# hitbc/panSVR

Measured on AMD Instinct MI355X. Metric: signal reads realigned/sec (150 bp PE); bit-exact CIGAR vs CPU ref, higher is better.
Workload: dtype u8/int32 (2-bit k-mers, 8-bit DP deltas, 32-bit scores); 1 GPU; configs[1]: 1000000 synthetic 150 bp PE signal read pairs per GPU vs 10000-anchor SV reference (11.8 Mbp), `panSVR aln` hot path; pairs_per_gpu=1000000, engines_per_gpu=1, in_process_rebases=0, index_hbm_bytes=2713674320, index_distribution=every rank uploads its own copy from host memory

## Files before the change

### include/psvr_engine.h

```cpp
#ifndef PSVR_ENGINE_H_
#define PSVR_ENGINE_H_

#include <stddef.h>
#include <stdint.h>

#ifdef __cplusplus
extern "C" {
#endif

#define PSVR_OK                0
#define PSVR_ERR_ARG           1
#define PSVR_ERR_UNSUPPORTED   2
#define PSVR_ERR_DEVICE        3
#define PSVR_ERR_NOMEM         4
#define PSVR_ERR_IO            5
#define PSVR_ERR_OVERFLOW      6

const char *psvr_last_error(void);
int psvr_device_count(void);
void *psvr_host_alloc(size_t bytes);
void psvr_host_free(void *p);
int psvr_device_warmup(int device, int n_streams);

#define PSVR_KSW_NEG_INF (-0x40000000)
#define PSVR_EZ_SCORE_ONLY  0x01
#define PSVR_EZ_RIGHT       0x02
#define PSVR_EZ_GENERIC_SC  0x04
#define PSVR_EZ_APPROX_MAX  0x08
#define PSVR_EZ_APPROX_DROP 0x10
#define PSVR_EZ_EXTZ_ONLY   0x40
#define PSVR_EZ_REV_CIGAR   0x80

typedef struct psvr_extz {
	int32_t max, zdropped;
	int32_t max_q, max_t;
	int32_t mqe, mqe_t;
	int32_t mte, mte_q;
	int32_t score;
	int32_t n_cigar;
	int32_t reach_end;
	int32_t reserved;
	int64_t cigar_off;
} psvr_extz_t;

typedef struct psvr_ksw_params {
	int8_t  m;
	int8_t  mat[25];
	int8_t  q, e, q2, e2;
	int32_t w;
	int32_t zdrop;
	int32_t end_bonus;
	int32_t flag;
} psvr_ksw_params_t;

static inline int64_t psvr_cigar_bound(int32_t qlen, int32_t tlen) { return (int64_t)qlen + tlen + 2; }

int psvr_extd2_batch(int device, int64_t n,
                     const uint8_t *qseq, const int64_t *q_off, const int32_t *qlen,
                     const uint8_t *tseq, const int64_t *t_off, const int32_t *tlen,
                     const psvr_ksw_params_t *par,
                     psvr_extz_t *ez, uint32_t *cigar_arena, int64_t cigar_cap);

int psvr_extz2_batch(int device, int64_t n,
                     const uint8_t *qseq, const int64_t *q_off, const int32_t *qlen,
                     const uint8_t *tseq, const int64_t *t_off, const int32_t *tlen,
                     const psvr_ksw_params_t *par,
                     psvr_extz_t *ez, uint32_t *cigar_arena, int64_t cigar_cap);

typedef struct psvr_dp_plan psvr_dp_plan_t;
int psvr_dp_plan_create(int device, int64_t n, const int32_t *qlen_host, const int32_t *tlen_host,
                        const psvr_ksw_params_t *par, int variant , psvr_dp_plan_t **plan);
int64_t psvr_dp_plan_workspace_bytes(const psvr_dp_plan_t *plan);
int psvr_dp_plan_launch(psvr_dp_plan_t *plan,
                        const uint8_t *d_qseq, const int64_t *d_q_off,
                        const uint8_t *d_tseq, const int64_t *d_t_off,
                        psvr_extz_t *d_ez, uint32_t *d_cigar_arena, void *d_work, void *stream);
int psvr_dp_plan_describe(const psvr_dp_plan_t *plan, char *buf, size_t buflen);
void psvr_dp_plan_destroy(psvr_dp_plan_t *plan);

typedef struct psvr_dp_regime {
	int32_t skip;
	int32_t swapped;
	int32_t nowrap_ok;
	int32_t zdrop_inert;
	int32_t long_thres;
	int32_t qe_shift;
} psvr_dp_regime_t;
int psvr_dp_regime(const psvr_ksw_params_t *par, int variant , psvr_dp_regime_t *out);


typedef struct psvr_index psvr_index_t;

typedef struct psvr_index_view {
	const uint64_t *ref_seq;  uint64_t n_ref_seq;
	const uint64_t *seq;      uint64_t n_seq;
	const uint64_t *seqf;     uint64_t n_seqf;
	const uint64_t *pos;      uint64_t n_pos;
	const uint64_t *posp;     uint64_t n_posp;
	const uint64_t *hash;     uint64_t n_hash;
	const uint32_t *kmer;     uint64_t n_kmer;
	const uint64_t *off;      uint64_t n_off;
	const char *chr_text;
	const char *const *header_names; int32_t n_header;
} psvr_index_view_t;

int psvr_index_create(const psvr_index_view_t *view, int device, psvr_index_t **out);
int psvr_index_create_from_device(const psvr_index_view_t *view, int device, psvr_index_t **out);
int psvr_index_load(const char *index_dir, const char *header_sam, int device, psvr_index_t **out);
int psvr_index_clone(const psvr_index_t *src, int device, psvr_index_t **out);
int psvr_index_build(const char *anchors_fa, const char *header_sam, int device, psvr_index_t **out);
void psvr_index_destroy(psvr_index_t *idx);
int64_t psvr_index_device_bytes(const psvr_index_t *idx);
int32_t psvr_index_n_anchor(const psvr_index_t *idx);
const char *psvr_index_sv_print_string(const psvr_index_t *idx, int32_t sv_id);
const char *psvr_index_sv_vcf_id(const psvr_index_t *idx, int32_t sv_id);

int psvr_seed_search_kmer_batch(const psvr_index_t *idx, int64_t n, const uint64_t *kmers, int64_t *range, uint8_t *found);
typedef struct psvr_vertex_mem {
	uint64_t uid;
	uint32_t seed_id;
	uint32_t read_pos, uni_pos_off, length, pos_n;
	uint32_t right_i;
} psvr_vertex_mem_t;
int psvr_seed_mem_batch(const psvr_index_t *idx, int64_t n, const uint64_t *kmer_index, const uint64_t *read_bits, int64_t n_words,
                        const int64_t *word_off, const uint32_t *read_off, const uint32_t *read_len, psvr_vertex_mem_t *out);

typedef struct psvr_engine psvr_engine_t;

typedef struct psvr_aln_params {
	int32_t match, mismatch, gap_open, gap_ex, gap_open2, gap_ex2, zdrop;
	int32_t normal_read_length, isize_min, isize_max;
	int32_t min_filter_score;
} psvr_aln_params_t;
void psvr_aln_params_default(psvr_aln_params_t *p);

typedef struct psvr_ori {
	int32_t  chr_id;
	uint32_t ref_bg, read_bg, align_score;
	uint8_t  mapq, direction , unmapped, reserved;
} psvr_ori_t;

#define PSVR_MAX_RESULT 12
typedef struct psvr_cand {
	uint32_t align_score, chain_score, ref_bg, read_bg;
	int32_t  chr_id, sv_id;
	uint32_t max_index;
	uint32_t n_cigar;
	int64_t  cigar_off;
	uint8_t  direction, mapq, reserved[6];
} psvr_cand_t;

typedef struct psvr_read_result {
	int32_t n_result;
	uint8_t unmapped, early_out, is_str, reserved;
	int32_t primary, secondary;
	int32_t has_mate, mate_chr_id;
	uint32_t mate_ref_bg;
	int32_t prim_sv_id, mate_sv_id;
	uint32_t n_seed[2];
	uint32_t reserved1;
	uint64_t seed_hash[2], chain_hash[2];
	psvr_cand_t cand[PSVR_MAX_RESULT];
} psvr_read_result_t;

typedef struct psvr_read_hdr {
	int32_t n_result;
	uint8_t unmapped, early_out, is_str, reserved;
	int32_t primary, secondary;
	int32_t has_mate, mate_chr_id;
	uint32_t mate_ref_bg;
	int32_t prim_sv_id, mate_sv_id;
	int32_t reserved2;
	int64_t cand_off;
} psvr_read_hdr_t;

typedef struct psvr_pair_result {
	int32_t max_score, cur_isize;
	int32_t proper, gain;
	int32_t max1, max2;
} psvr_pair_result_t;

int psvr_engine_create(const psvr_index_t *idx, const psvr_aln_params_t *par, psvr_engine_t **out);
void psvr_engine_destroy(psvr_engine_t *eng);
int psvr_engine_align_batch(psvr_engine_t *eng, int64_t n_pairs, const char *bases, const int64_t *base_off,
                            const psvr_ori_t *ori, psvr_read_result_t *reads, psvr_pair_result_t *pairs,
                            uint32_t *cigar, int64_t cigar_cap, int trace);
int psvr_engine_upload(psvr_engine_t *eng, int64_t n_pairs, const char *bases, const int64_t *base_off, const psvr_ori_t *ori);
int psvr_engine_run(psvr_engine_t *eng, int trace, void *stream);
int psvr_engine_download(psvr_engine_t *eng, psvr_read_result_t *reads, psvr_pair_result_t *pairs,
                         uint32_t *cigar, int64_t cigar_cap, int64_t *cigar_used);
int psvr_engine_download_compact(psvr_engine_t *eng, psvr_read_hdr_t *hdr, psvr_pair_result_t *pairs,
                                 psvr_cand_t *cands, int64_t cand_cap, int64_t *cand_used,
                                 uint32_t *cigar, int64_t cigar_cap, int64_t *cigar_used);
int psvr_engine_set_stream_pos(psvr_engine_t *eng, const int64_t pos[3]);
int psvr_engine_stream_end(psvr_engine_t *eng, int64_t end[3]);
int psvr_engine_rebase(psvr_engine_t *eng, const int64_t pos[3], void *stream);
int psvr_engine_stats(const psvr_engine_t *eng, char *buf, size_t buflen);

typedef struct psvr_fastq psvr_fastq_t;
typedef struct psvr_fastq_info {
	int64_t n_pairs, used_bytes, total_bases, n_lines;
	int32_t stop;
	int32_t reserved;
} psvr_fastq_info_t;
int  psvr_fastq_create(int device, psvr_fastq_t **out);
int  psvr_fastq_parse(psvr_fastq_t *fq, const char *text, int64_t n_bytes, int at_end,
                      int64_t max_pairs, int64_t max_bases, psvr_fastq_info_t *info);
int  psvr_fastq_download(const psvr_fastq_t *fq, uint64_t *line_start, uint16_t *name_end,
                         int64_t *base_off, psvr_ori_t *ori, char *bases);
int  psvr_engine_upload_fastq(psvr_engine_t *eng, const psvr_fastq_t *fq, int64_t first_pair, int64_t n_pairs);
void psvr_fastq_destroy(psvr_fastq_t *fq);

typedef struct psvr_bam_emit psvr_bam_emit_t;
typedef struct psvr_bam_emit_info { int64_t n_bytes, n_records, n_written_pairs, n_declined_pairs; } psvr_bam_emit_info_t;
#define PSVR_EMIT_NOT_ORI 1
int  psvr_bam_emit_create(const psvr_index_t *idx, psvr_bam_emit_t **out);
int  psvr_bam_emit_results(psvr_bam_emit_t *em, const psvr_fastq_t *fq, int64_t first_pair, int64_t n_pairs,
                           const psvr_read_hdr_t *hdr, const psvr_pair_result_t *pairs, const psvr_cand_t *cands, int64_t n_cands,
                           const uint32_t *cigar, int64_t n_cigar, int32_t flags, psvr_bam_emit_info_t *info);
int  psvr_bam_emit_engine(psvr_bam_emit_t *em, psvr_engine_t *eng, const psvr_fastq_t *fq, int32_t flags, psvr_bam_emit_info_t *info);
int  psvr_bam_emit_download(const psvr_bam_emit_t *em, void *bytes, int64_t cap, int64_t *pair_off, uint8_t *pair_state);
void psvr_bam_emit_destroy(psvr_bam_emit_t *em);

int64_t psvr_bgzf_bound(int64_t n_bytes);
int psvr_bgzf_compress(int device, const void *in, int64_t n_bytes, void *out, int64_t out_cap, int64_t *out_bytes);

int64_t psvr_bgzf_members_bound(int64_t n_bytes, int32_t member_bytes);
int psvr_bgzf_compress_members(int device, const void *in, int64_t n_bytes, int32_t member_bytes,
                               void *out, int64_t out_cap, int64_t *out_bytes,
                               int64_t *member_off, int64_t member_cap, int64_t *n_members);

int psvr_bgzf_decompress(int device, const void *in, int64_t n_bytes, int64_t *in_used,
                         void *out, int64_t out_cap, int64_t *out_bytes,
                         int64_t *member_off, int64_t member_cap, int64_t *n_members, int64_t *bad_member);

int psvr_sort_order_u64(int device, int64_t n, const uint64_t *keys, uint32_t *order);

#ifdef __cplusplus
}
#endif
#endif
```

### pansvr_amd/csrc/aln_device.h

```cpp
#pragma once
#include <stdint.h>
#include "../../include/psvr_engine.h"

#if defined(__HIPCC__)
#include <hip/hip_runtime.h>
#define PSVR_HD __host__ __device__ __forceinline__
#define PSVR_HDN __host__ __device__
#else
#define PSVR_HD inline
#define PSVR_HDN
#endif

namespace psvr {

static const int kLenKmer = 20, kSeedStep = 5, kUniPosNMax = 32;
static const int kMaxOut = 6;
static const int kMaxReadLen = 1600;
static const int kFwd = 1, kRev = 0;
static const int kSegMax = 160;
static const int kCigMax = 256;
static const int kMemSlot = 32;

struct SvDev { uint32_t chr_id; uint32_t st_pos; int32_t end_offset; int32_t pad; };

// ... 14 lines not shown
};

PSVR_HD void hash_pair(const DevIndex &ix, uint64_t h, uint64_t &lo, uint64_t &hi);

struct VMem { uint64_t uid; uint32_t seed_id, read_pos, uni_pos_off, length, pos_n, pad; };
struct VU { uint64_t uid; uint32_t read_pos, uni_pos_off, length1, length2, pos_n, cov; };
struct USeed { uint32_t read_begin, read_end, seed_id, ref_begin, ref_end, cov; };
struct PathN { int32_t dist, pre_node; uint32_t brk; uint32_t used; };

static const int kArenaTopStride = 32, kArenaMaxShards = 16;
template <class T> struct Arena {
	T *base;
	unsigned long long *top;
	unsigned long long cap;
	int *overflow;
	unsigned int nshard;
};

PSVR_HD unsigned long long atomic_bump(unsigned long long *p, unsigned long long n)
{
#if defined(__HIP_DEVICE_COMPILE__)
	return atomicAdd(p, n);
#else
	unsigned long long o = *p;
	*p += n;
	return o;
#endif
}

template <class T> PSVR_HD long long arena_alloc(const Arena<T> &a, unsigned long long n)
{
#if defined(__HIP_DEVICE_COMPILE__)
	if (a.nshard > 1) {
		const unsigned long long cap_s = a.cap / a.nshard;
		for (unsigned int k = 0; k < a.nshard; ++k) {
			const unsigned long long s = (blockIdx.x + k) % a.nshard;
			if (k && a.top[s * kArenaTopStride] + n > cap_s) continue;
			const unsigned long long o = atomic_bump(a.top + s * kArenaTopStride, n);
			if (o + n <= cap_s) return (long long)(s * cap_s + o);
		}
		*a.overflow = 1;
		return -1;
	}
#endif
	unsigned long long o = atomic_bump(a.top, n);
	if (o + n > a.cap) { *a.overflow = 1; return -1; }
	return (long long)o;
}

struct Strand {
	long long mem_off; uint32_t mem_n;
	long long us_off;  uint32_t us_n;
	uint64_t seed_hash, chain_hash;
};

struct ChainCand {
	uint32_t chain_score, max_index, read_bg, ref_bg;
	int32_t chr_id;
	int32_t direction;
};

struct Seg {
	int32_t kind;
	int32_t a, b;
};

struct DpDesc {
	int32_t read, strand;
	int32_t q_st, qlen;
	uint32_t ref_st; int32_t tlen;
	int32_t type;
	int32_t pad;
};

struct CandWork {
	int32_t read, k;
	int32_t n_seg;
	int32_t read_score;
	int32_t rba;
	int32_t bad;
	long long seg_off;
};

struct Ctx {
	DevIndex idx;
	psvr_aln_params_t par;
	int8_t mat[25];
	long long n_pairs;
	const char *bases; const long long *base_off; const psvr_ori_t *ori;
	int32_t lmax;
	int32_t wmax;
	const int32_t *grand; long long grand_n; long long grand_base;
	const int32_t *hrand[2]; long long hrand_n; long long hrand_base[2];
	long long n_slots;
	const int32_t *src;
	long long *poff;
	int32_t *rcnt;
	long long *hoff; int32_t *hcnt;
	const uint8_t *force;
	uint8_t *active; uint8_t *unmapped; uint8_t *is_str; uint8_t *has_n4;
	uint8_t *has_mem;
	int32_t *str_list; unsigned int *str_cnt;
	int32_t *read_l;
	uint8_t *bin;
	uint64_t *rb;
	uint8_t *seed_list;
	Strand *strand;
	ChainCand *ccand; int32_t *n_ccand;
	psvr_read_hdr_t *rh; psvr_pair_result_t *pres;
	psvr_cand_t *cand;
	Arena<VMem> mem; Arena<USeed> us; PathN *path;
	Arena<Seg> seg; Arena<DpDesc> dp; Arena<CandWork> cw; Arena<uint32_t> cig;
	const psvr_extz_t *dp_ez; const uint32_t *dp_cig;
	const uint8_t *tseq_in; int32_t *stale_open;
	int32_t *any_h;
	int32_t trace;
	int32_t *err;
	unsigned long long *stats;
};

enum { ST_PROBES = 0, ST_HITS, ST_SEEDS, ST_DP, ST_SIMPLE, ST_CELLS, ST_READS, ST_CAND, ST_N };

PSVR_HD void stat_add(const Ctx &c, int k, unsigned long long v)
{
	if (!c.stats) return;
#if defined(__HIP_DEVICE_COMPILE__)
	atomicAdd(c.stats + k, v);
#else
	c.stats[k] += v;
#endif
}

PSVR_HD long long src_read(const Ctx &c, long long read)
{
	return c.src ? (long long)c.src[read >> 1] * 2 + (read & 1) : read;
}

PSVR_HD uint64_t fnv1a(uint64_t h, uint64_t v)
{
	for (int i = 0; i < 8; ++i) { h ^= (v >> (8 * i)) & 0xff; h *= 1099511628211ULL; }
	return h;
}

PSVR_HD bool bucket_occupied(const DevIndex &ix, uint64_t h)
{
#ifdef PSVR_EMU_SPARSE_HASH
	(void)ix, (void)h;
	return true;
#else
	return !ix.occ || ((ix.occ[h >> 5] >> (h & 31)) & 1u);
#endif
}

PSVR_HD void bloom_slot(uint64_t kmer, uint32_t shift, uint64_t &word, uint64_t &mask)
{
	const uint64_t h = kmer * 0x9E3779B97F4A7C15ull;
	const uint64_t g = (h ^ (h >> 32)) * 0xD6E8FEB86659FD93ull;
	word = h >> shift;
	mask = (1ull << (g >> 58)) | (1ull << ((g >> 52) & 63)) | (1ull << ((g >> 46) & 63));
}
PSVR_HD bool kmer_maybe_present(const DevIndex &ix, uint64_t kmer)
{
#ifdef PSVR_EMU_SPARSE_HASH
	(void)ix, (void)kmer;
	return true;
#else
	if (ix.bloom) {
		uint64_t w, m;
		bloom_slot(kmer, ix.bloom_shift, w, m);
		return (ix.bloom[w] & m) == m;
	}
	return bucket_occupied(ix, kmer >> 12);
#endif
}

PSVR_HD void hash_pair(const DevIndex &ix, uint64_t h, uint64_t &lo, uint64_t &hi)
{
#ifdef PSVR_EMU_SPARSE_HASH
	auto at = [&](uint64_t x) {
		uint64_t l = 0, r = ix.sp_n;
		while (l < r) { uint64_t m = (l + r) >> 1; if (ix.sp_id[m] < x) l = m + 1; else r = m; }
		return l < ix.sp_n ? ix.sp_start[l] : ix.n_kmer;
	};
	lo = at(h), hi = at(h + 1);
#else
	lo = ix.hash[h], hi = ix.hash[h + 1];
#endif
}

PSVR_HD int base_at(const uint64_t *w, uint64_t i) { return (int)((w[i >> 5] >> ((31 - (i & 0x1f)) << 1)) & 3); }

PSVR_HD uint64_t window32(const uint64_t *w, uint64_t i)
{
	uint64_t k = i >> 5, sh = (i & 31) << 1;
	uint64_t a = w[k];
	return sh ? (a << sh) | (w[k + 1] >> (64 - sh)) : a;
}
PSVR_HD int mismatches_packed(const uint64_t *A, uint64_t ia, const uint64_t *B, uint64_t ib, int len, int cap)
{
	int nm = 0;
	for (int j = 0; j < len && nm < cap; j += 128) {
		const uint64_t ka = (ia + (uint64_t)j) >> 5, kb = (ib + (uint64_t)j) >> 5;
		const unsigned sa = (unsigned)((ia + (uint64_t)j) & 31) << 1, sb = (unsigned)((ib + (uint64_t)j) & 31) << 1;
		const int rem = len - j, nw = rem >= 128 ? 4 : (rem + 31) >> 5;
		uint64_t wa[5], wb[5];
#if defined(__HIP_DEVICE_COMPILE__)
#pragma unroll
#endif
		for (int q = 0; q < 5; ++q) { const bool in = q <= nw; wa[q] = in ? A[ka + q] : 0, wb[q] = in ? B[kb + q] : 0; }
#if defined(__HIP_DEVICE_COMPILE__)
#pragma unroll
#endif
		for (int q = 0; q < 4; ++q) {
			if (q >= nw) break;
			const uint64_t xa = sa ? (wa[q] << sa) | (wa[q + 1] >> (64 - sa)) : wa[q], xb = sb ? (wb[q] << sb) | (wb[q + 1] >> (64 - sb)) : wb[q];
			uint64_t x = xa ^ xb;
			x = (x | (x >> 1)) & 0x5555555555555555ull;
			const int r = rem - 32 * q;
			if (r < 32) x &= ~0ull << ((32 - r) << 1);
#if defined(__HIP_DEVICE_COMPILE__)
			nm += __popcll(x);
#else
			nm += __builtin_popcountll(x);
#endif
		}
	}
	return nm < cap ? nm : cap;
}

PSVR_HDN inline void prep_read(const Ctx &c, long long read)
{
	const long long sr = src_read(c, read);
	const psvr_ori_t &o = c.ori[sr];
	const int L = (int)(c.base_off[sr + 1] - c.base_off[sr]);
	c.read_l[read] = L;
	bool unm = o.unmapped != 0;
	if ((uint32_t)o.chr_id > 24u) unm = true;
	c.unmapped[read] = unm;
	c.is_str[read] = 0, c.has_mem[read] = 0;
	long long item = (read >> 1) * 3 + (read & 1);
	c.rcnt[item] = 0;
	c.hcnt[read] = 0;
	c.n_ccand[read] = 0;
	for (int s = 0; s < 2; ++s) { Strand &st = c.strand[read * 2 + s]; st.mem_n = st.us_n = 0; st.mem_off = st.us_off = 0; st.seed_hash = st.chain_hash = 1469598103934665603ULL; }
	if (L > kMaxReadLen || L < kLenKmer) { c.active[read] = 0; if (L > kMaxReadLen) *c.err = 1; return; }
	if (!unm && o.align_score == (uint32_t)(L * c.par.match)) { c.active[read] = 0; return; }
	c.active[read] = 1;
	const char *s = c.bases + c.base_off[sr];
	uint8_t *b0 = c.bin + (read * 2) * (long long)c.lmax, *b1 = b0 + c.lmax;
	uint64_t *w0 = c.rb + (read * 2) * (long long)c.wmax, *w1 = w0 + c.wmax;
	for (int i = 0; i < c.wmax; ++i) w0[i] = 0, w1[i] = 0;
	long long ro = c.poff[read >> 1] + ((read & 1) ? c.rcnt[(read >> 1) * 3] : 0);
	int draws = 0;
	for (int i = 0; i < L; ++i) {
		char ch = s[i];
		if (ch == 'N') {
			long long k = ro + draws - c.grand_base;
			int32_t r;
			if (c.force && draws < (int)c.force[4 * read]) r = c.force[4 * read + 1 + draws];
			else r = (k >= 0 && k < c.grand_n) ? c.grand[k] : (*c.err = 2, 0);
			ch = "ACGT"[r % 4];
			++draws;
		}
		uint8_t code = (ch == 'C' || ch == 'c') ? 1 : (ch == 'G' || ch == 'g') ? 2 : (ch == 'T' || ch == 't') ? 3 : (ch == 'n') ? 4 : 0;
		b0[i] = code;
		b1[L - 1 - i] = code ^ 3;
	}
	for (int i = 0; i < L; ++i) {
		w0[i >> 5] |= ((uint64_t)b0[i]) << ((31 - (i & 0x1f)) << 1);
		w1[i >> 5] |= ((uint64_t)b1[i]) << ((31 - (i & 0x1f)) << 1);
	}
	c.rcnt[item] = draws;
	{ uint8_t any4 = 0; for (int i = 0; i < L; ++i) any4 |= b0[i] > 3; c.has_n4[read] = any4; }
	stat_add(c, ST_READS, 1);
}

PSVR_HD uint64_t get_kmer(uint32_t off, const uint64_t *rb)
{
	uint32_t w = off >> 5, iw = off & 0x1f;
	uint64_t full = (rb[w] << (iw << 1)) | (iw == 0 ? 0 : (rb[w + 1] >> ((32 - iw) << 1)));
	return full >> ((32 - kLenKmer) << 1);
}

PSVR_HDN inline void str_detect(const Ctx &c, long long read)
{
	if (!c.active[read]) return;
	const int L = c.read_l[read];
	const uint64_t *rb = c.rb + (read * 2) * (long long)c.wmax;
	uint8_t *sl = c.seed_list + read * (long long)c.lmax;
	const uint32_t kn = L - kLenKmer + 1;
	uint32_t distinct = 0;
	for (uint32_t i = 0; i < kn; ++i) {
		uint64_t ki = get_kmer(i, rb);
		bool first = true;
		for (uint32_t j = 0; j < i; ++j) if (get_kmer(j, rb) == ki) { first = false; break; }
		distinct += first;
	}
	if (!(distinct < kn - 15)) { c.is_str[read] = 0; return; }
	c.is_str[read] = 1;
	for (uint32_t i = 0; i < kn; ++i) {
		uint64_t ki = get_kmer(i, rb);
		int cnt = 0;
		for (uint32_t j = 0; j < kn; ++j) cnt += get_kmer(j, rb) == ki;
		sl[i] = cnt >= 4 ? 0 : 1;
	}
	int bg = 0, ed = 0;
	for (uint32_t o = 0; o < (uint32_t)kSeedStep; ++o) {
		bg += sl[o] == 0, ed += sl[L - kLenKmer - o] == 0;
		sl[o] += 2, sl[L - kLenKmer - o] += 4;
	}
	if (bg < kSeedStep && ed < kSeedStep) {
		int tot = 0;
		for (uint32_t o = 0; tot < kSeedStep && o < kn; ++o) {
			if (sl[o] > 0) continue;
			sl[o] += 8, tot++;
		}
	}
}

PSVR_HD uint8_t seed_list_at(const uint8_t *sl, int len, int rev, int i)
{
	if (!rev) return sl[i];
	if (!(len & 1) && (i == len / 2 || i == len / 2 - 1)) return sl[i];
	return sl[len - 1 - i];
}

PSVR_HD int clz64(uint64_t x)
{
#if defined(__HIP_DEVICE_COMPILE__)
	return __clzll((long long)x);
#else
	return __builtin_clzll(x);
#endif
}
PSVR_HD int ctz64(uint64_t x)
{
#if defined(__HIP_DEVICE_COMPILE__)
	return __ffsll((unsigned long long)x) - 1;
#else
	return __builtin_ctzll(x);
#endif
}
PSVR_HD uint32_t match_right(const uint64_t *A, uint64_t ia, const uint64_t *B, uint64_t ib, uint32_t max)
{
	uint32_t n = 0;
	while (n < max) {
		const uint64_t ka = (ia + n) >> 5;
		const unsigned sa = (unsigned)((ia + n) & 31) << 1;
		const uint32_t rem = max - n;
		const int nw = rem >= 128 ? 4 : (int)((rem + 31) >> 5);
		uint64_t wa[5];
#if defined(__HIP_DEVICE_COMPILE__)
#pragma unroll
#endif
		for (int q = 0; q < 5; ++q) wa[q] = (q < nw || (q == nw && sa != 0)) ? A[ka + q] : 0;
#if defined(__HIP_DEVICE_COMPILE__)
#pragma unroll
#endif
		for (int q = 0; q < 4; ++q) {
			if (q >= nw) break;
			const uint64_t xa = sa ? (wa[q] << sa) | (wa[q + 1] >> (64 - sa)) : wa[q];
			uint64_t x = xa ^ window32(B, ib + n + 32u * (uint32_t)q);
			x = (x | (x >> 1)) & 0x5555555555555555ull;
			const uint32_t left = rem - 32u * (uint32_t)q, lim = left < 32 ? left : 32;
			if (x) { const uint32_t k = (uint32_t)clz64(x) >> 1; return n + 32u * (uint32_t)q + (k < lim ? k : lim); }
		}
		n += rem < 128 ? rem : 128;
	}
	return max;
}
PSVR_HD uint32_t match_left(const uint64_t *A, uint64_t ia, const uint64_t *B, uint64_t ib, uint32_t max)
{
	uint32_t n = 0;
	while (n < max) {
		uint32_t lim = max - n < 32 ? max - n : 32;
		uint64_t x = window32(A, ia - n - lim) ^ window32(B, ib - n - lim);
		x = (x | (x >> 1)) & 0x5555555555555555ull;
		if (lim < 32) x &= ~0ull << ((32 - lim) << 1);
		if (x) { uint32_t k = ((uint32_t)ctz64(x) - ((32 - lim) << 1)) >> 1; return n + k; }
		n += lim;
	}
	return max;
}

PSVR_HD uint32_t probe_kmer(const DevIndex &ix, uint64_t kmer, uint64_t &first_hit)
{
	const uint64_t key = kmer & 0xfff, h = kmer >> 12;
	uint64_t lo, hi;
	hash_pair(ix, h, lo, hi);
	long long l = 0, r = (long long)(hi - lo) - 1, first = -1, last = -1;
	const uint32_t *v = ix.kmer + lo;
	while (l <= r) {
		long long m = (l + r) / 2;
		uint32_t t = v[m] >> 4;
		if (t == key) {
			first = last = m;
			long long sl2 = l, sr = m - 1;
			while (sl2 <= sr) { long long sm = (sl2 + sr) / 2; uint32_t t2 = v[sm] >> 4; if (t2 == key) first = sm, sr = sm - 1; else if (t2 > key) sr = sm - 1; else sl2 = sm + 1; }
			sl2 = m + 1, sr = r;
			while (sl2 <= sr) { long long sm = (sl2 + sr) / 2; uint32_t t2 = v[sm] >> 4; if (t2 == key) last = sm, sl2 = sm + 1; else if (t2 > key) sr = sm - 1; else sl2 = sm + 1; }
			break;
		} else if (t > key) r = m - 1;
		else l = m + 1;
	}
	if (first < 0) return 0;
	first_hit = lo + (uint64_t)first;
	return (uint32_t)(last - first + 1);
}

PSVR_HDN inline HitRec hit_record(const DevIndex &ix, uint64_t hit)
{
	HitRec h;
	const uint64_t kp = ix.off[hit];
	long long lo2 = 0, hi2 = (long long)ix.n_seqf - 1, uid = -1;
	if (ix.uid_hint) {
		const uint64_t b = kp >> ix.uid_shift;
		lo2 = (long long)ix.uid_hint[b], hi2 = (long long)ix.uid_hint[b + 1];
	}
	while (lo2 <= hi2) {
		long long mid = (lo2 + hi2) >> 1;
		uint64_t sv = ix.seqf[mid];
		if (kp < sv) hi2 = mid - 1;
		else if (kp > sv) lo2 = mid + 1;
		else { uid = mid; break; }
	}
	if (uid < 0) uid = hi2;
	const uint64_t f0 = ix.seqf[uid], f1 = ix.seqf[uid + 1];
	h.kp = kp, h.uid = (uint32_t)uid, h.ul = (uint32_t)(kp - f0), h.ur = (uint32_t)(f1 - (kp + kLenKmer));
	h.pos_n = (uint32_t)(ix.posp[uid + 1] - ix.posp[uid]), h.pad[0] = h.pad[1] = 0;
	return h;
}
PSVR_HD uint32_t mem_for_hit(const DevIndex &ix, uint64_t hit, const uint64_t *rb, uint32_t off, int L, VMem &m)
{
	const HitRec h = ix.hitrec ? ix.hitrec[hit] : hit_record(ix, hit);
	const uint64_t kp = h.kp, uid = h.uid;
	const uint32_t ul = h.ul, ur = h.ur;
	const uint32_t lmax = ul < off ? ul : off, rmax0 = (uint32_t)(L - (int)off - kLenKmer), rmax = ur < rmax0 ? ur : rmax0;
	const uint32_t li = 1 + match_left(ix.seq, kp, rb, off, lmax);
	const uint32_t ri = 1 + match_right(ix.seq, kp + kLenKmer, rb, (uint64_t)off + kLenKmer, rmax);
	m.uid = (uint64_t)uid, m.seed_id = 0, m.read_pos = off + 1 - li, m.uni_pos_off = ul + 1 - li;
	m.length = kLenKmer + li + ri - 2, m.pos_n = h.pos_n, m.pad = 0;
	return ri;
}

template <bool LOCAL> PSVR_HD void seed_strand_t(const Ctx &c, long long rs, const uint64_t *rb_local)
{
	const long long read = rs >> 1;
	const int rev = (int)(rs & 1);
	if (!c.active[read]) return;
	const int L = c.read_l[read];
	const uint64_t *rb = LOCAL ? rb_local : c.rb + rs * (long long)c.wmax;
	const uint8_t *sl = c.seed_list + read * (long long)c.lmax;
	const bool is_str = c.is_str[read] != 0;
	const uint32_t kn = L - kLenKmer + 1;
	const DevIndex &ix = c.idx;
	long long base = rs * (long long)kMemSlot;
	uint32_t total = 0, probes = 0;
	for (int pass = 0; pass < 3; ++pass) {
		if (pass == 1) continue;
		uint32_t n = 0, msr = 0, off = 0, nh = 0;
		uint64_t kmer = 0, first_hit = 0;
		int stage = 0;
		for (;;) {
			while (stage != 2 && off < kn) {
				while (off < kn) {
					if (off + kLenKmer - 1 <= msr || (is_str && seed_list_at(sl, (int)kn, rev, off) == 0)) { off += kSeedStep; continue; }
					if (pass == 0) ++probes;
					kmer = get_kmer(off, rb);
					if (kmer_maybe_present(ix, kmer)) { stage = 1; break; }
					off += kSeedStep;
				}
				if (stage != 1) break;
				nh = probe_kmer(ix, kmer, first_hit);
				if (nh == 0 || nh > (uint32_t)kUniPosNMax) { off += kSeedStep; stage = 0; }
				else stage = 2;
			}
			if (stage != 2) break;
			uint32_t mri = 1;
			for (uint64_t hit = first_hit; hit < first_hit + nh; ++hit) {
				VMem m;
				const uint32_t ri = mem_for_hit(ix, hit, rb, off, L, m);
				m.seed_id = n;
				if (pass == 2 || n < (uint32_t)kMemSlot) c.mem.base[base + n] = m;
				++n;
				if (ri > mri) mri = ri;
			}
			msr = off + kLenKmer + mri - 1;
			off += kSeedStep;
			stage = 0;
		}
		if (pass == 0) {
			total = n;
			if (n <= (uint32_t)kMemSlot) break;
			base = arena_alloc(c.mem, n);
			if (base < 0) return;
		}
	}
	Strand &st = c.strand[rs];
	st.mem_off = base, st.mem_n = total;
	if (total) c.has_mem[read] = 1;
	if (c.stats) { stat_add(c, ST_PROBES, probes); stat_add(c, ST_HITS, total); }
}
PSVR_HDN inline void seed_strand(const Ctx &c, long long rs) { seed_strand_t<false>(c, rs, nullptr); }

template <class T, class Less> PSVR_HD void stable_sort(T *a, T *tmp, uint32_t n, Less less)
{
	if (n < 2) return;
	if (n <= 16) {
		for (uint32_t i = 1; i < n; ++i) {
			T x = a[i];
			uint32_t j = i;
			while (j > 0 && less(x, a[j - 1])) { a[j] = a[j - 1]; --j; }
			a[j] = x;
		}
		return;
	}
	T *src = a, *dst = tmp;
	for (uint32_t w = 1; w < n; w <<= 1) {
		for (uint32_t lo = 0; lo < n; lo += 2 * w) {
			uint32_t mid = lo + w < n ? lo + w : n, hi = lo + 2 * w < n ? lo + 2 * w : n;
			uint32_t i = lo, j = mid, k = lo;
			while (i < mid && j < hi) { if (less(src[j], src[i])) dst[k++] = src[j++]; else dst[k++] = src[i++]; }
			while (i < mid) dst[k++] = src[i++];
			while (j < hi) dst[k++] = src[j++];
		}
		T *t = src; src = dst; dst = t;
	}
	if (src != a) for (uint32_t i = 0; i < n; ++i) a[i] = src[i];
}

PSVR_HDN inline void chain_strand(const Ctx &c, long long rs, int &hdraw_total)
{
	const long long read = rs >> 1;
	const int rev = (int)(rs & 1);
	if (!c.active[read]) return;
	Strand &st = c.strand[rs];
	const uint32_t mem_i = st.mem_n;
	VMem *vm = c.mem.base + st.mem_off;
	const DevIndex &ix = c.idx;
	if (mem_i > 1) {
		VMem *mtmp = nullptr;
		if (mem_i > 16) {
			long long t = arena_alloc(c.mem, mem_i);
			if (t < 0) return;
			mtmp = c.mem.base + t;
		}
		stable_sort(vm, mtmp, mem_i, [](const VMem &a, const VMem &b) { return a.uid != b.uid ? a.uid < b.uid : a.read_pos < b.read_pos; });
	}
	long long ubase = 0;
	uint32_t total = 0;
	const long long hro = c.hoff[read] + hdraw_total;
	int hdraw = 0;
	for (int pass = 0; pass < 2; ++pass) {
		uint32_t n = 0, vu_i = 0;
		hdraw = 0;
		bool stop = false;
		uint32_t j = 0;
		while (j < mem_i && !stop) {
			VU u;
			if (mem_i == 1) {
				const VMem &m = vm[0];
				u.uid = m.uid, u.read_pos = m.read_pos, u.uni_pos_off = m.uni_pos_off, u.length1 = u.length2 = m.length, u.pos_n = m.pos_n, u.cov = m.length;
				j = 1;
			} else {
				uint32_t s1 = j, cov = vm[s1].length;
				const uint64_t uid_t = vm[s1].uid;
				j++;
				while (j < mem_i && uid_t == vm[j].uid && vm[j].uni_pos_off > vm[j - 1].uni_pos_off) {
					int diff = (int)(vm[j].read_pos - vm[j - 1].read_pos - vm[j - 1].length);
					if (diff > 3) break;
					int ce = (int)((vm[j].uni_pos_off - vm[j - 1].uni_pos_off) - (vm[j].read_pos - vm[j - 1].read_pos));
					if ((ce < 0 ? -ce : ce) < 1) { cov += (diff > 0) ? vm[j].length : (uint32_t)(diff + (int)vm[j].length); ++j; }
					else break;
				}
				uint32_t e1 = j - 1;
				u.uid = vm[s1].uid, u.read_pos = vm[s1].read_pos, u.uni_pos_off = vm[s1].uni_pos_off, u.pos_n = vm[s1].pos_n, u.cov = cov;
				if (s1 == e1) u.length1 = u.length2 = vm[s1].length;
				else {
					u.length1 = vm[e1].read_pos + vm[e1].length - vm[s1].read_pos;
					u.length2 = vm[e1].uni_pos_off + vm[e1].length - vm[s1].uni_pos_off;
				}
			}
			uint32_t cnt = u.pos_n;
			bool sample = false;
			if (u.pos_n > 500) {
				if (u.pos_n > 8000) { stop = true; break; }
				cnt = 500, sample = true;
			}
			for (uint32_t k = 0; k < cnt; ++k) {
				uint32_t m = k;
				if (sample) {
					long long q = hro + hdraw - c.hrand_base[read & 1];
					int32_t rv = (q >= 0 && q < c.hrand_n) ? c.hrand[read & 1][q] : (*c.err = 3, 0);
					m = (uint32_t)rv % u.pos_n;
					++hdraw;
				}
				if (pass == 1) {
					USeed &s = c.us.base[ubase + n];
					s.seed_id = vu_i, s.read_begin = u.read_pos, s.read_end = u.read_pos + u.length1 - 1;
					s.ref_begin = (uint32_t)(ix.pos[m + ix.posp[u.uid]] + u.uni_pos_off - 1);
					s.ref_end = s.ref_begin + u.length2 - 1, s.cov = u.cov;
				}
				++n;
			}
			++vu_i;
		}
		if (pass == 0) {
			total = n;
			if (n == 0) break;
			ubase = arena_alloc(c.us, 2ull * n);
			if (ubase < 0) return;
		}
	}
	(void)rev;
	st.us_off = ubase, st.us_n = total;
	hdraw_total += hdraw;
	if (total == 0) return;
	USeed *v = c.us.base + ubase;
	PathN *pa = c.path + ubase;
	stable_sort(v, v + total, total, [](const USeed &a, const USeed &b) { return a.ref_end != b.ref_end ? a.ref_end < b.ref_end : a.ref_begin < b.ref_begin; });
	const bool is_str = c.is_str[read] != 0;
	const int max_ref_dis = is_str ? 400 : 50, max_read_dis = is_str ? 400 : 50;
// ... 1147 lines not shown
```

### pansvr_amd/csrc/engine.hip

```cpp
#include <hip/hip_runtime.h>
#include <algorithm>
#include <cstring>
#include <mutex>
#include <string>
#include <thread>
#include <vector>
#include "common.h"
#include "engine_core.h"
#include "bam_emit_hooks.h"
#include "fastq_parsed.h"
#include "host_io.h"
#include "index_build.h"
#include "ksw_device.h"
#include "ksw_launch.h"
#include "scan.h"

namespace psvr {

int dp_params(const psvr_ksw_params_t *par, int variant, DpParams *P);

static const int kBlock = 256;
static inline unsigned grid_for(long long n, int block = kBlock) { return (unsigned)((n + block - 1) / block); }

__device__ __forceinline__ long long pair_of(const int32_t *work, long long i) { return work ? (long long)work[i] : i; }
// ... 1744 lines not shown
	bi.ref_seq.resize(bi.ref_seq.size());
	psvr_index_view_t v;
	memset(&v, 0, sizeof v);
	v.ref_seq = bi.ref_seq.data(), v.n_ref_seq = bi.ref_seq.size(), v.seq = bi.seqb.data(), v.n_seq = bi.seqb.size();
	v.seqf = bi.seqf.data(), v.n_seqf = bi.seqf.size(), v.pos = bi.pos.data(), v.n_pos = bi.pos.size(), v.posp = bi.posp.data(), v.n_posp = bi.posp.size();
	v.hash = nullptr, v.n_hash = ((uint64_t)1 << 28) + 1, v.kmer = bi.kmer.data(), v.n_kmer = bi.kmer.size(), v.off = bi.off.data(), v.n_off = bi.off.size();
	std::vector<uint32_t> sid(bi.hash_sparse_id.size()), scn(bi.hash_sparse_cnt.size());
	for (size_t i = 0; i < sid.size(); ++i) sid[i] = (uint32_t)bi.hash_sparse_id[i], scn[i] = (uint32_t)bi.hash_sparse_cnt[i];
	int rc = index_upload(ix, &v, sid.data(), scn.data(), (long long)sid.size());
	if (rc) { delete ix; return rc; }
	*out = ix;
	return PSVR_OK;
}

extern "C" int psvr_index_load(const char *dir, const char *header_sam, int device, psvr_index_t **out)
{
	if (!dir || !header_sam || !out) return set_error(PSVR_ERR_ARG, "psvr_index_load: null argument");
	if (psvr_device_count() <= 0) return set_error(PSVR_ERR_DEVICE, "no HIP device visible: the engine has no CPU path");
	psvr_index *ix = new psvr_index;
	ix->device = device;
	std::string err;
	ix->host.defer_dense = true;
	if (!ix->host.load_dir(dir, header_sam, &err)) { delete ix; return set_error(PSVR_ERR_IO, "%s", err.c_str()); }
	HostIndex &h = ix->host;
	psvr_index_view_t v;
	memset(&v, 0, sizeof v);
	v.ref_seq = h.ref_seq.data(), v.n_ref_seq = h.ref_seq.size(), v.seq = h.seq.data(), v.n_seq = h.seq.size();
	v.seqf = h.seqf.data(), v.n_seqf = h.seqf.size(), v.pos = h.pos.data(), v.n_pos = h.pos.size(), v.posp = h.posp.data(), v.n_posp = h.posp.size();
	v.hash = h.hash.data(), v.n_hash = h.hash.size(), v.kmer = h.kmer.data(), v.n_kmer = h.kmer.size(), v.off = h.off.data(), v.n_off = h.off.size();
	int rc;
	if (!h.sparse_pairs.empty()) {
		const size_t ns = h.sparse_pairs.size() / 2;
		std::vector<uint32_t> sid(ns), scn(ns);
		for (size_t i = 0; i < ns; ++i) sid[i] = h.sparse_pairs[2 * i], scn[i] = h.sparse_pairs[2 * i + 1];
		{
			unsigned long long tot = 0;
			bool ok = true;
			for (size_t i = 0; i < ns && ok; ++i) { ok = sid[i] < (1u << 28) && (i == 0 || sid[i] > sid[i - 1]); tot += scn[i]; }
			if (!ok || tot != (unsigned long long)h.kmer.size()) { delete ix; return set_error(PSVR_ERR_IO, "unipath_g.hash.sparse: bucket ids must be < 4^14 and ascending, counts must add up to the %zu entries of unipath_g.kmer", h.kmer.size()); }
		}
		v.hash = nullptr, v.n_hash = ((uint64_t)1 << 28) + 1;
		rc = index_upload(ix, &v, sid.data(), scn.data(), (long long)ns);
		std::vector<uint32_t>().swap(h.sparse_pairs);
	} else rc = index_upload(ix, &v);
	std::vector<uint64_t>().swap(h.hash);
	if (rc) { delete ix; return rc; }
	*out = ix;
	return PSVR_OK;
}

extern "C" int psvr_index_clone(const psvr_index_t *src, int device, psvr_index_t **out)
{
	if (!src || !out) return set_error(PSVR_ERR_ARG, "psvr_index_clone: null argument");
	psvr_index *ix = new psvr_index;
	ix->device = device;
	ix->host = src->host;
	hipError_t he = hipSetDevice(device);
	auto cp = [&](DevBuf &d, const DevBuf &s0) {
		if (he != hipSuccess || !s0.p) return;
		he = d.alloc(s0.bytes);
		if (he == hipSuccess) he = hipMemcpyPeer(d.p, device, s0.p, src->device, s0.bytes);
		ix->bytes += (int64_t)s0.bytes;
	};
	cp(ix->ref_seq, src->ref_seq), cp(ix->seq, src->seq), cp(ix->seqf, src->seqf), cp(ix->pos, src->pos), cp(ix->posp, src->posp), cp(ix->hash, src->hash);
	cp(ix->off, src->off), cp(ix->kmer, src->kmer), cp(ix->chr_end, src->chr_end), cp(ix->chr_idx, src->chr_idx), cp(ix->sv, src->sv), cp(ix->occ, src->occ), cp(ix->uid_hint, src->uid_hint), cp(ix->bloom, src->bloom), cp(ix->hitrec, src->hitrec);
	if (he == hipSuccess) he = hipDeviceSynchronize();
	if (he != hipSuccess) { delete ix; return set_error(PSVR_ERR_DEVICE, "psvr_index_clone: %s", hipGetErrorString(he)); }
	DevIndex &d = ix->dev;
	d = src->dev;
	d.ref_seq = ix->ref_seq.as<uint64_t>(), d.seq = ix->seq.as<uint64_t>(), d.seqf = ix->seqf.as<uint64_t>(), d.pos = ix->pos.as<uint64_t>();
	d.posp = ix->posp.as<uint64_t>(), d.hash = ix->hash.as<uint64_t>(), d.off = ix->off.as<uint64_t>(), d.kmer = ix->kmer.as<uint32_t>();
	d.chr_end_n = ix->chr_end.as<uint32_t>(), d.chr_search_index = ix->chr_idx.as<uint32_t>(), d.sv = ix->sv.as<SvDev>();
	d.occ = ix->occ.as<uint32_t>(), d.uid_hint = ix->uid_hint.as<uint32_t>();
	if (src->bloom.p) d.bloom = ix->bloom.as<uint64_t>();
	if (src->hitrec.p) d.hitrec = ix->hitrec.as<HitRec>();
	*out = ix;
	return PSVR_OK;
}

extern "C" void psvr_index_destroy(psvr_index_t *ix) { delete ix; }
extern "C" int64_t psvr_index_device_bytes(const psvr_index_t *ix) { return ix ? ix->bytes : 0; }
extern "C" int32_t psvr_index_n_anchor(const psvr_index_t *ix) { return ix ? ix->host.chr_file_n : 0; }
extern "C" const char *psvr_index_sv_print_string(const psvr_index_t *ix, int32_t sv)
{
	return ix && sv >= 0 && sv < (int)ix->host.svh.size() ? ix->host.svh[sv].vcf_print_string.c_str() : nullptr;
}
extern "C" const char *psvr_index_sv_vcf_id(const psvr_index_t *ix, int32_t sv)
{
	return ix && sv >= 0 && sv < (int)ix->host.svh.size() ? ix->host.svh[sv].vcf_id.c_str() : nullptr;
}

__global__ __launch_bounds__(kBlock) void k_b3_search_kmer(DevIndex ix, long long n, const uint64_t *kmers, long long *range, uint8_t *found)
{
	const long long i = blockIdx.x * (long long)blockDim.x + threadIdx.x;
	if (i >= n) return;
	const uint64_t kmer = kmers[i] & 0xffffffffffull;
	uint64_t first = 0;
	const uint32_t nh = kmer_maybe_present(ix, kmer) ? probe_kmer(ix, kmer, first) : 0;
	found[i] = nh != 0;
	range[2 * i] = nh ? (long long)first : 0, range[2 * i + 1] = nh ? (long long)(first + nh - 1) : -1;
}
__global__ __launch_bounds__(kBlock) void k_b3_mem(DevIndex ix, long long n, const uint64_t *kmer_index, const uint64_t *read_bits, const long long *word_off, const uint32_t *read_off,
                                                   const uint32_t *read_len, psvr_vertex_mem_t *out)
{
	const long long i = blockIdx.x * (long long)blockDim.x + threadIdx.x;
	if (i >= n) return;
	VMem m;
	const uint32_t ri = mem_for_hit(ix, kmer_index[i], read_bits + word_off[i], read_off[i], (int)read_len[i], m);
	psvr_vertex_mem_t &o = out[i];
	o.uid = m.uid, o.seed_id = 0, o.read_pos = m.read_pos, o.uni_pos_off = m.uni_pos_off, o.length = m.length, o.pos_n = m.pos_n, o.right_i = ri;
}

extern "C" int psvr_seed_search_kmer_batch(const psvr_index_t *ix, int64_t n, const uint64_t *kmers, int64_t *range, uint8_t *found)
{
	if (!ix || n < 0 || (n && (!kmers || !range || !found))) return set_error(PSVR_ERR_ARG, "psvr_seed_search_kmer_batch: bad argument");
	if (n == 0) return PSVR_OK;
	PSVR_HIP(hipSetDevice(ix->device));
	DevBuf dk, dr, df;
	PSVR_HIP(dk.alloc((size_t)n * 8)); PSVR_HIP(dr.alloc((size_t)n * 16)); PSVR_HIP(df.alloc((size_t)n));
	PSVR_HIP(hipMemcpy(dk.p, kmers, (size_t)n * 8, hipMemcpyHostToDevice));
	hipLaunchKernelGGL(k_b3_search_kmer, dim3(grid_for(n)), dim3(kBlock), 0, nullptr, ix->dev, (long long)n, dk.as<uint64_t>(), dr.as<long long>(), df.as<uint8_t>());
	PSVR_HIP(hipGetLastError());
	PSVR_HIP(hipMemcpy(range, dr.p, (size_t)n * 16, hipMemcpyDeviceToHost));
	PSVR_HIP(hipMemcpy(found, df.p, (size_t)n, hipMemcpyDeviceToHost));
	return PSVR_OK;
}

extern "C" int psvr_seed_mem_batch(const psvr_index_t *ix, int64_t n, const uint64_t *kmer_index, const uint64_t *read_bits, int64_t n_words, const int64_t *word_off,
                                   const uint32_t *read_off, const uint32_t *read_len, psvr_vertex_mem_t *out)
{
	if (!ix || n < 0 || n_words < 0 || (n && (!kmer_index || !read_bits || !word_off || !read_off || !read_len || !out))) return set_error(PSVR_ERR_ARG, "psvr_seed_mem_batch: bad argument");
	if (n == 0) return PSVR_OK;
	const uint64_t n_index = ix->off.bytes / 8;
	for (int64_t i = 0; i < n; ++i) {
		const int64_t words = ((int64_t)read_len[i] + 31) / 32 + 1;
		if (kmer_index[i] >= n_index || word_off[i] < 0 || word_off[i] + words > n_words || read_len[i] < (uint32_t)kLenKmer || read_off[i] + (uint32_t)kLenKmer > read_len[i])
			return set_error(PSVR_ERR_ARG, "psvr_seed_mem_batch: item %lld is out of range (index entry, word window or read offset)", (long long)i);
	}
	PSVR_HIP(hipSetDevice(ix->device));
	DevBuf dk, db, dw, dro, drl, dout;
	PSVR_HIP(dk.alloc((size_t)n * 8)); PSVR_HIP(db.alloc((size_t)(n_words + 2) * 8)); PSVR_HIP(dw.alloc((size_t)n * 8)); PSVR_HIP(dro.alloc((size_t)n * 4)); PSVR_HIP(drl.alloc((size_t)n * 4));
	PSVR_HIP(dout.alloc((size_t)n * sizeof(psvr_vertex_mem_t)));
	PSVR_HIP(hipMemset((char *)db.p + (size_t)n_words * 8, 0, 16));
	PSVR_HIP(hipMemcpy(dk.p, kmer_index, (size_t)n * 8, hipMemcpyHostToDevice)); PSVR_HIP(hipMemcpy(db.p, read_bits, (size_t)n_words * 8, hipMemcpyHostToDevice));
	PSVR_HIP(hipMemcpy(dw.p, word_off, (size_t)n * 8, hipMemcpyHostToDevice)); PSVR_HIP(hipMemcpy(dro.p, read_off, (size_t)n * 4, hipMemcpyHostToDevice));
	PSVR_HIP(hipMemcpy(drl.p, read_len, (size_t)n * 4, hipMemcpyHostToDevice));
	hipLaunchKernelGGL(k_b3_mem, dim3(grid_for(n)), dim3(kBlock), 0, nullptr, ix->dev, (long long)n, dk.as<uint64_t>(), db.as<uint64_t>(), dw.as<long long>(), dro.as<uint32_t>(), drl.as<uint32_t>(),
	                   dout.as<psvr_vertex_mem_t>());
	PSVR_HIP(hipGetLastError());
	PSVR_HIP(hipMemcpy(out, dout.p, (size_t)n * sizeof(psvr_vertex_mem_t), hipMemcpyDeviceToHost));
	return PSVR_OK;
}

extern "C" int psvr_device_warmup(int device, int n_streams)
{
	if (device < 0 || device >= 64 || n_streams < 1) return set_error(PSVR_ERR_ARG, "psvr_device_warmup: bad argument");
	if (n_streams > 16) n_streams = 16;
	std::thread([device, n_streams]() {
		if (hipSetDevice(device) != hipSuccess) return;
		std::vector<hipStream_t> got;
		void *h = nullptr, *d = nullptr;
		const bool buf = hipHostMalloc(&h, 4096, hipHostMallocDefault) == hipSuccess && hipMalloc(&d, 4096) == hipSuccess;
		if (buf) memset(h, 0, 4096);
		for (int i = 0; i < n_streams; ++i) {
			hipStream_t s = nullptr;
			if (hipStreamCreateWithFlags(&s, hipStreamNonBlocking) != hipSuccess) break;
			if (buf) (void)hipMemcpyAsync(d, h, 4096, hipMemcpyHostToDevice, s), (void)hipMemsetAsync(d, 0, 4096, s), (void)hipMemcpyAsync(h, d, 4096, hipMemcpyDeviceToHost, s);
			(void)hipStreamSynchronize(s);
			got.push_back(s);
		}
		if (h) (void)hipHostFree(h);
		if (d) (void)hipFree(d);
		(void)hipGetLastError();
		StreamPool &P = stream_pool();
		std::lock_guard<std::mutex> lk(P.mu);
		for (hipStream_t s : got) P.idle[device].push_back(s);
	}).detach();
	return PSVR_OK;
}

struct psvr_engine {
	const psvr_index *ix;
	GpuBE be;
	EngineCore<GpuBE, GpuBE> core;
	bool committed = true;
	DevBuf full_out, cmp_cnt_c, cmp_cnt_w, cmp_off_c, cmp_off_w, cmp_hdr, cmp_cand, cmp_cig;
	bool compact_valid = false;
	long long compact_nc = 0, compact_nw = 0;
	hipStream_t own = nullptr;
	const psvr_fastq *src_fq = nullptr;
	int64_t src_first = 0, src_n = 0;
	uint64_t src_generation = 0;
	bool ran = false;
	explicit psvr_engine(const psvr_index *i) : ix(i), core(be) {}
};

extern "C" void psvr_aln_params_default(psvr_aln_params_t *p) { if (p) aln_params_default(p); }

extern "C" int psvr_engine_create(const psvr_index_t *ix, const psvr_aln_params_t *par, psvr_engine_t **out)
{
	if (!ix || !par || !out) return set_error(PSVR_ERR_ARG, "psvr_engine_create: null argument");
	PSVR_HIP(hipSetDevice(ix->device));
	psvr_engine *e = new psvr_engine(ix);
	e->own = stream_pool().get(ix->device);
	e->be.stream = e->own, e->be.device = ix->device;
	e->core.init(ix->dev, *par);
	*out = e;
	return PSVR_OK;
}

extern "C" void psvr_engine_destroy(psvr_engine_t *e)
{
	if (!e) return;
	(void)hipSetDevice(e->ix->device);
	const int dev = e->ix->device;
	hipStream_t own = e->own;
	delete e;
	stream_pool().put(dev, own);
}

static int engine_status(psvr_engine *e, int rc)
{
	if (e->be.last != hipSuccess) { hipError_t x = e->be.last; e->be.last = hipSuccess; return set_error(PSVR_ERR_DEVICE, "HIP error: %s", hipGetErrorString(x)); }
	if (rc) return set_error(rc, "%s", e->core.err.empty() ? psvr_last_error() : e->core.err.c_str());
	return PSVR_OK;
}

extern "C" int psvr_engine_upload(psvr_engine_t *e, int64_t n_pairs, const char *bases, const int64_t *base_off, const psvr_ori_t *ori)
{
	if (!e || n_pairs < 0 || (n_pairs && (!bases || !base_off || !ori))) return set_error(PSVR_ERR_ARG, "psvr_engine_upload: bad argument");
	PSVR_HIP(hipSetDevice(e->ix->device));
	e->be.stream = e->own;
	if (!e->committed) { e->core.commit(); e->committed = true; }
	e->compact_valid = false;
	e->src_fq = nullptr, e->ran = false;
	int rc = e->core.upload(n_pairs, bases, base_off, ori);
	return engine_status(e, rc);
}

extern "C" int psvr_engine_upload_fastq(psvr_engine_t *e, const psvr_fastq_t *fq, int64_t first_pair, int64_t n_pairs)
{
	if (psvr_device_count() <= 0) return set_error(PSVR_ERR_DEVICE, "no HIP device visible: the engine has no CPU path");
	if (!e || !fq || !fq->valid || first_pair < 0 || n_pairs < 0 || first_pair + n_pairs > fq->last.n_pairs) return set_error(PSVR_ERR_ARG, "psvr_engine_upload_fastq: bad argument");
	if (fq->device != e->ix->device)
		return set_error(PSVR_ERR_ARG, "psvr_engine_upload_fastq: the text was parsed on device %d, the engine runs on device %d (the bases would have to travel between them)", fq->device, e->ix->device);
	PSVR_HIP(hipSetDevice(e->ix->device));
	e->be.stream = e->own;
	if (!e->committed) { e->core.commit(); e->committed = true; }
	e->compact_valid = false;
	e->src_fq = nullptr, e->ran = false;
	const int64_t *off = fq->base_off.as<int64_t>() + 2 * first_pair;
	long long b0 = 0, b1 = fq->last.total_bases;
	const bool whole = first_pair == 0 && n_pairs == fq->last.n_pairs;
	if (!whole && n_pairs > 0 && !e->be.d2h({{&b0, off, 8}, {&b1, off + 2 * n_pairs, 8}})) return engine_status(e, PSVR_ERR_DEVICE);
	const int rc = e->core.upload_device(n_pairs, fq->bases.as<char>(), off, fq->ori.as<psvr_ori_t>() + 2 * first_pair, b0, b1 - b0);
	const int st = engine_status(e, rc);
	if (!st) e->src_fq = fq, e->src_first = first_pair, e->src_n = n_pairs, e->src_generation = fq->generation;
	return st;
}

extern "C" int psvr_engine_run(psvr_engine_t *e, int trace, void *stream)
{
	if (!e) return set_error(PSVR_ERR_ARG, "psvr_engine_run: null engine");
	PSVR_HIP(hipSetDevice(e->ix->device));
	e->be.stream = stream ? (hipStream_t)stream : e->own;
	e->be.timing = (trace & 4) != 0;
	e->be.timed.clear();
	e->compact_valid = false;
	int rc = e->core.run(trace & 1, (trace & 2) != 0);
	hipError_t s = hipStreamSynchronize(e->be.stream);
	if (s != hipSuccess) e->be.note(s);
	e->be.synced();
	e->be.collect_timing();
	e->committed = false;
	const int st = engine_status(e, rc);
	e->ran = st == PSVR_OK;
	return st;
}

extern "C" int psvr_engine_set_stream_pos(psvr_engine_t *e, const int64_t pos[3])
{
	if (!e || !pos) return set_error(PSVR_ERR_ARG, "psvr_engine_set_stream_pos: null argument");
	PSVR_HIP(hipSetDevice(e->ix->device));
	e->core.have_run = false, e->committed = true;
	e->core.grand_pos = pos[0], e->core.hrand_pos[0] = pos[1], e->core.hrand_pos[1] = pos[2];
	return PSVR_OK;
}

extern "C" int psvr_engine_stream_end(psvr_engine_t *e, int64_t end[3])
{
	if (!e || !end) return set_error(PSVR_ERR_ARG, "psvr_engine_stream_end: null argument");
	PSVR_HIP(hipSetDevice(e->ix->device));
	long long t[3];
	e->core.stream_end(t);
	end[0] = t[0], end[1] = t[1], end[2] = t[2];
	return engine_status(e, PSVR_OK);
}

extern "C" int psvr_engine_rebase(psvr_engine_t *e, const int64_t pos[3], void *stream)
{
	if (!e || !pos) return set_error(PSVR_ERR_ARG, "psvr_engine_rebase: null argument");
	PSVR_HIP(hipSetDevice(e->ix->device));
	e->be.stream = stream ? (hipStream_t)stream : e->own;
	e->compact_valid = false;
	int rc = e->core.rebase(pos[0], pos[1], pos[2], e->core.c.trace, false);
	hipError_t s = hipStreamSynchronize(e->be.stream);
// ... 132 lines not shown
```

Baseline: 356.5 million reads/s.

## Probe canonical bloom once per k-mer pair and share answers across strand lanes

The bloom filter is now keyed on the canonical (min of forward and reverse-complement) 20-mer, with separate bit masks for the two orientations, so one word fetch answers presence for a k-mer and its reverse complement. Forward and reverse strand threads of a read split the seed offsets between them, batch five bloom loads at a time to overlap memory latency, and exchange the other strand's answers through a lane shuffle. The seeding loop then reads a precomputed answer bitmask instead of probing the filter per offset. This adds reverse-complement arithmetic and assumes the paired strand lanes are adjacent and both active. It also adds a host API to read back the filter.

```diff
diff --git a/include/psvr_engine.h b/include/psvr_engine.h
--- a/include/psvr_engine.h
+++ b/include/psvr_engine.h
@@ -124,6 +124,7 @@
 } psvr_vertex_mem_t;
 int psvr_seed_mem_batch(const psvr_index_t *idx, int64_t n, const uint64_t *kmer_index, const uint64_t *read_bits, int64_t n_words,
                         const int64_t *word_off, const uint32_t *read_off, const uint32_t *read_len, psvr_vertex_mem_t *out);
+int psvr_index_bloom_read(const psvr_index_t *idx, uint64_t *words, int64_t n_words, int64_t *n_words_out, uint32_t *shift_out);
 
 typedef struct psvr_engine psvr_engine_t;
 
diff --git a/pansvr_amd/csrc/aln_device.h b/pansvr_amd/csrc/aln_device.h
--- a/pansvr_amd/csrc/aln_device.h
+++ b/pansvr_amd/csrc/aln_device.h
@@ -190,12 +190,39 @@
 #endif
 }
 
+PSVR_HD uint64_t rc20(uint64_t x)
+{
+	x = ~x;
+	x = ((x >> 2) & 0x3333333333333333ull) | ((x & 0x3333333333333333ull) << 2);
+	x = ((x >> 4) & 0x0f0f0f0f0f0f0f0full) | ((x & 0x0f0f0f0f0f0f0f0full) << 4);
+	return __builtin_bswap64(x) >> (64 - 2 * kLenKmer);
+}
+PSVR_HD uint64_t bloom_hash(uint64_t c, uint32_t shift, uint64_t &word)
+{
+	const uint64_t h = c * 0x9E3779B97F4A7C15ull;
+	word = h >> shift;
+	return (h ^ (h >> 32)) * 0xD6E8FEB86659FD93ull;
+}
+PSVR_HD void bloom_masks(uint64_t g, uint64_t &lo, uint64_t &hi)
+{
+	lo = (1ull << (g >> 58)) | (1ull << ((g >> 52) & 63)) | (1ull << ((g >> 46) & 63));
+	hi = (1ull << ((g >> 40) & 63)) | (1ull << ((g >> 34) & 63)) | (1ull << ((g >> 28) & 63));
+}
+PSVR_HD void bloom_slot2(uint64_t kmer, uint32_t shift, uint64_t &word, uint64_t &mask, uint64_t &mask_rc)
+{
+	const uint64_t r = rc20(kmer);
+	uint64_t lo, hi;
+	bloom_masks(bloom_hash(kmer < r ? kmer : r, shift, word), lo, hi);
+	mask = kmer <= r ? lo : hi, mask_rc = r <= kmer ? lo : hi;
+}
 PSVR_HD void bloom_slot(uint64_t kmer, uint32_t shift, uint64_t &word, uint64_t &mask)
 {
-	const uint64_t h = kmer * 0x9E3779B97F4A7C15ull;
-	const uint64_t g = (h ^ (h >> 32)) * 0xD6E8FEB86659FD93ull;
-	word = h >> shift;
-	mask = (1ull << (g >> 58)) | (1ull << ((g >> 52) & 63)) | (1ull << ((g >> 46) & 63));
+	uint64_t mrc;
+	bloom_slot2(kmer, shift, word, mask, mrc);
+}
+PSVR_HD uint32_t bloom_answers(uint64_t w, uint64_t mask, uint64_t mask_rc)
+{
+	return (uint32_t)((w & mask) == mask) | ((uint32_t)((w & mask_rc) == mask_rc) << 1);
 }
 PSVR_HD bool kmer_maybe_present(const DevIndex &ix, uint64_t kmer)
 {
@@ -481,6 +508,52 @@
 	return ri;
 }
 
+static const int kSeedPairBatch = 5;
+PSVR_HD bool seed_pair_applies(const DevIndex &ix, int L)
+{
+	return ix.bloom && (L - kLenKmer) % kSeedStep == 0 && L - kLenKmer <= 63 * kSeedStep;
+}
+PSVR_HD void seed_pair_half(const DevIndex &ix, const uint64_t *rb, int T, int rev, uint64_t &own, uint64_t &other)
+{
+	const int t0 = rev ? (T & 1) : 0, cnt = rev ? T >> 1 : (T + 1) >> 1;
+	own = other = 0;
+	for (int j0 = 0; j0 < cnt; j0 += kSeedPairBatch) {
+		uint64_t w[kSeedPairBatch], g[kSeedPairBatch];
+		uint32_t canon = 0, pal = 0;
+#if defined(__HIP_DEVICE_COMPILE__)
+#pragma unroll
+#endif
+		for (int q = 0; q < kSeedPairBatch; ++q) {
+			const bool in = j0 + q < cnt;
+			const uint64_t x = get_kmer((uint32_t)((in ? t0 + 2 * (j0 + q) : t0) * kSeedStep), rb), r = rc20(x);
+			canon |= (uint32_t)(x <= r) << q, pal |= (uint32_t)(x == r) << q;
+			uint64_t word;
+			g[q] = bloom_hash(x < r ? x : r, ix.bloom_shift, word);
+			w[q] = in ? ix.bloom[word] : 0;
+		}
+#if defined(__HIP_DEVICE_COMPILE__)
+#pragma unroll
+#endif
+		for (int q = 0; q < kSeedPairBatch; ++q) {
+			if (j0 + q >= cnt) break;
+			const int t = t0 + 2 * (j0 + q);
+			uint64_t lo, hi;
+			bloom_masks(g[q], lo, hi);
+			const bool cn = (canon >> q) & 1, pl = (pal >> q) & 1;
+			const uint32_t a = bloom_answers(w[q], cn ? lo : hi, (pl || !cn) ? lo : hi);
+			own |= (uint64_t)(a & 1) << t, other |= (uint64_t)(a >> 1) << (T - 1 - t);
+		}
+	}
+}
+#if defined(__HIP_DEVICE_COMPILE__)
+__device__ __forceinline__ uint64_t seed_pair_answers(const DevIndex &ix, const uint64_t *rb, int T, int rev)
+{
+	uint64_t own, other;
+	seed_pair_half(ix, rb, T, rev, own, other);
+	return own | (uint64_t)__shfl_xor((unsigned long long)other, 1);
+}
+#endif
+
 template <bool LOCAL> PSVR_HD void seed_strand_t(const Ctx &c, long long rs, const uint64_t *rb_local)
 {
 	const long long read = rs >> 1;
@@ -494,6 +567,14 @@
 	const DevIndex &ix = c.idx;
 	long long base = rs * (long long)kMemSlot;
 	uint32_t total = 0, probes = 0;
+	bool paired = false;
+	uint64_t answers = 0;
+#if defined(__HIP_DEVICE_COMPILE__)
+	if (LOCAL && seed_pair_applies(ix, L) && !c.has_n4[read]) {
+		answers = seed_pair_answers(ix, rb, (L - kLenKmer) / kSeedStep + 1, rev);
+		paired = true;
+	}
+#endif
 	for (int pass = 0; pass < 3; ++pass) {
 		if (pass == 1) continue;
 		uint32_t n = 0, msr = 0, off = 0, nh = 0;
@@ -505,7 +586,7 @@
 					if (off + kLenKmer - 1 <= msr || (is_str && seed_list_at(sl, (int)kn, rev, off) == 0)) { off += kSeedStep; continue; }
 					if (pass == 0) ++probes;
 					kmer = get_kmer(off, rb);
-					if (kmer_maybe_present(ix, kmer)) { stage = 1; break; }
+					if (paired ? (answers >> (off / kSeedStep)) & 1 : kmer_maybe_present(ix, kmer)) { stage = 1; break; }
 					off += kSeedStep;
 				}
 				if (stage != 1) break;
diff --git a/pansvr_amd/csrc/engine.hip b/pansvr_amd/csrc/engine.hip
--- a/pansvr_amd/csrc/engine.hip
+++ b/pansvr_amd/csrc/engine.hip
@@ -1920,6 +1920,19 @@
 	return PSVR_OK;
 }
 
+extern "C" int psvr_index_bloom_read(const psvr_index_t *ix, uint64_t *words, int64_t n_words, int64_t *n_words_out, uint32_t *shift_out)
+{
+	if (!ix || n_words < 0 || (n_words && !words)) return set_error(PSVR_ERR_ARG, "psvr_index_bloom_read: bad argument");
+	const int64_t have = (int64_t)(ix->bloom.bytes / 8);
+	if (n_words_out) *n_words_out = have;
+	if (shift_out) *shift_out = ix->dev.bloom_shift;
+	if (n_words == 0) return PSVR_OK;
+	if (n_words != have) return set_error(PSVR_ERR_ARG, "psvr_index_bloom_read: the filter has %lld words", (long long)have);
+	PSVR_HIP(hipSetDevice(ix->device));
+	PSVR_HIP(hipMemcpy(words, ix->bloom.p, (size_t)have * 8, hipMemcpyDeviceToHost));
+	return PSVR_OK;
+}
+
 extern "C" int psvr_device_warmup(int device, int n_streams)
 {
 	if (device < 0 || device >= 64 || n_streams < 1) return set_error(PSVR_ERR_ARG, "psvr_device_warmup: bad argument");
```

New measurement: 373.3 million reads/s (median of 6 runs). 4.7% higher.
